# genomematt/xenomapper

Hardware: AMD Instinct MI355X
Metric: read-pairs/sec classified (higher is better)
Workload: dtype int32; 1 GPU; configs[1]: 50000000 PE 2x150 pairs/GPU, AS/XS, liberal, HBM-resident; pairs_per_gpu=50000000, step=xm_classify_compact_dev: classify+count, scan, scatter (3 launches)

## Files before the change

### xenomapper_amd/csrc/xm_kernels.hip

```cpp
#include <hip/hip_runtime.h>
#include <stdint.h>
#include <stdlib.h>

#include "xm_kernels.h"

namespace xm {

template <typename T>
__device__ __forceinline__ uint32_t mapping_state(T a1, T x1, T a2, T x2, T m)
{
    const bool low1 = a1 <= m;
    const bool low2 = a2 <= m;
    const bool prim = (a1 > m) && (low2 || a1 > a2);
    const bool sec  = (a2 > m) && (low1 || a2 > a1);
    const bool spec1 = (x1 == T(0)) || (a1 > x1);
    const bool spec2 = (x2 == T(0)) || (a2 > x2);
    uint32_t s = 6u;
    s = sec ? (spec2 ? 1u : 3u) : s;
    s = (a1 == a2) ? 4u : s;
    s = prim ? (spec1 ? 0u : 2u) : s;
    s = (low1 && low2) ? 5u : s;
    return s;
}

// ... 5 lines not shown
    const bool spec1 = (x1 == 0) || (a1 > x1);
    const bool spec2 = (x2 == 0) || (a2 > x2);
    uint32_t s = spec2 ? 1u : 3u;
    s = (gt || lt) ? s : 4u;
    s = (!low1 && (low2 || gt)) ? (spec1 ? 0u : 2u) : s;
    s = (low1 && low2) ? 5u : s;
    return s;
}

__device__ __forceinline__ uint32_t bin_of_code(int mode, uint32_t c)
{
    const uint32_t f = (c >> 3) & 7u, r = c & 7u;
    const uint32_t lo = f < r ? f : r;
    const uint32_t hi = f < r ? r : f;
    uint32_t b;
    if (mode == XM_MODE_SE) {
        b = r > 6u ? 6u : r;
    } else if (mode == XM_MODE_PE_LIBERAL) {
        b = lo;
    } else {
        b = (hi == 5u) ? 5u
          : ((hi == 4u) || (((f ^ r) & 1u) != 0u)) ? 4u
          : lo;
    }
    if (mode != XM_MODE_SE) b = (hi > 5u) ? 6u : b;
    return (c == XM_NO_UNIT) ? 7u : b;
}

template <typename T> struct Vec4;
typedef int32_t v4i32 __attribute__((ext_vector_type(4)));
typedef int32_t v4i32_a4 __attribute__((ext_vector_type(4), aligned(4)));
typedef double  v4f64 __attribute__((ext_vector_type(4)));
template <> struct Vec4<int32_t> { typedef v4i32 type; };
template <> struct Vec4<double>  { typedef v4f64 type; };

template <typename T> __device__ __forceinline__ T absent_value();
template <> __device__ __forceinline__ int32_t absent_value<int32_t>() { return INT32_MIN; }
template <> __device__ __forceinline__ double  absent_value<double>()  { return -__builtin_huge_val(); }

template <typename T, bool NT, bool FULL = false>
__device__ __forceinline__ void load4(const T *__restrict__ col, uint64_t r0, uint64_t n, T out[4])
{
    typedef typename Vec4<T>::type V;
    if (FULL || r0 + 4 <= n) {
        const V *p = reinterpret_cast<const V *>(col + r0);
        const V v = NT ? __builtin_nontemporal_load(p) : *p;
        out[0] = v.x; out[1] = v.y; out[2] = v.z; out[3] = v.w;
    } else {
#pragma unroll
        for (int j = 0; j < 4; ++j) out[j] = (r0 + j < n) ? col[r0 + j] : absent_value<T>();
    }
}

template <typename T, bool NT>
__device__ __forceinline__ void load4_wg(const T *__restrict__ wg, uint32_t byte_off, T out[4])
{
    typedef typename Vec4<T>::type V;
    const V *p = reinterpret_cast<const V *>(reinterpret_cast<const char *>(wg) + byte_off);
    const V v = NT ? __builtin_nontemporal_load(p) : *p;
    out[0] = v.x; out[1] = v.y; out[2] = v.z; out[3] = v.w;
}

__device__ __forceinline__ uint32_t wave_scan_incl(uint32_t v)
{
    v += (uint32_t)__builtin_amdgcn_update_dpp(0, (int)v, 0x111, 0xf, 0xf, false);
    v += (uint32_t)__builtin_amdgcn_update_dpp(0, (int)v, 0x112, 0xf, 0xf, false);
    v += (uint32_t)__builtin_amdgcn_update_dpp(0, (int)v, 0x114, 0xf, 0xf, false);
    v += (uint32_t)__builtin_amdgcn_update_dpp(0, (int)v, 0x118, 0xf, 0xf, false);
    v += (uint32_t)__builtin_amdgcn_update_dpp(0, (int)v, 0x142, 0xa, 0xf, false);
    v += (uint32_t)__builtin_amdgcn_update_dpp(0, (int)v, 0x143, 0xc, 0xf, false);
    return v;
}

__device__ __forceinline__ uint32_t lane_value(uint32_t v, int lane)
{
    return (uint32_t)__builtin_amdgcn_readlane((int)v, lane);
}

__device__ __forceinline__ void lds_settle()
{
    asm volatile("s_waitcnt lgkmcnt(0)" ::: "memory");
}

#define XM_HREP 8
#define XM_COUNT_LDS_WORDS (64 * XM_HREP + 16)

struct CountSink {
    uint32_t *gran_counts;
    uint32_t *part_tot;
    unsigned long long *counts_rep;
    uint8_t *bins4;
    uint32_t gran_stride;
    int mode;
    uint32_t blk0;
};

__device__ __forceinline__ void count_flush(uint32_t *lds, uint32_t granule, const CountSink &sink)
{
    const uint32_t lane = threadIdx.x & 63u;
    uint32_t *misc = lds + 64 * XM_HREP;
    const uint4 h0 = *reinterpret_cast<const uint4 *>(lds + lane * XM_HREP);
    const uint4 h1 = *reinterpret_cast<const uint4 *>(lds + lane * XM_HREP + 4);
    const uint32_t s = h0.x + h0.y + h0.z + h0.w + h1.x + h1.y + h1.z + h1.w;
    if (s != 0u) {
        atomicAdd(&sink.counts_rep[(granule % XM_COUNT_REPLICAS) * 64u + lane], (unsigned long long)s);
        atomicAdd(&misc[8u + bin_of_code(sink.mode, lane)], s);
    }
    lds_settle();
    if (lane < 8u) {
        const uint32_t v = misc[8u + lane];
        sink.gran_counts[(uint64_t)lane * sink.gran_stride + granule] = v;
        if (v != 0u) atomicAdd(&sink.part_tot[((granule & (XM_PART_REPLICAS - 1u)) * 8u + lane) * XM_PART_STRIDE + granule / XM_PART_GRAN], v);
    }
}

template <int BLOCK>
__device__ __forceinline__ void count_units(const uint32_t c[4], uint32_t *lds, const CountSink &sink)
{
    const uint32_t lane = threadIdx.x & 63u;
    const uint32_t rep = lane & (XM_HREP - 1u);
#pragma unroll
    for (int j = 0; j < 4; ++j) {
        const bool unit = c[j] != XM_NO_UNIT;
        if (__ballot(unit) == 0ull) continue;
        if (unit) atomicAdd(&lds[(c[j] & 63u) * XM_HREP + rep], 1u);
    }
    lds_settle();
    uint32_t arrived = 0;
    if (lane == 0u) arrived = atomicAdd(&lds[64 * XM_HREP], 1u);
    arrived = (uint32_t)__builtin_amdgcn_readfirstlane((int)arrived);
    if (arrived != (uint32_t)(BLOCK / 64 - 1)) return;
    lds_settle();
    count_flush(lds, blockIdx.x + sink.blk0, sink);
}

template <int MODE, bool HAS6>
__device__ __forceinline__ uint32_t unit_bin(uint32_t c)
{
    if (MODE == XM_MODE_SE) return c == XM_NO_UNIT ? 7u : (c & 7u);
    const uint32_t f = (c >> 3) & 7u, r = c & 7u;
    const uint32_t lo = f < r ? f : r, hi = f < r ? r : f;
    uint32_t b = lo;
    if (MODE == XM_MODE_PE_CONSERVATIVE) {
        b = (((f ^ r) & 1u) != 0u || hi == 4u) ? 4u : b;
        b = (hi == 5u) ? 5u : b;
    }
    if (HAS6) b = (hi > 5u) ? 6u : b;
    return c == XM_NO_UNIT ? 7u : b;
}

template <int MODE, bool HAS6>
__device__ __forceinline__ uint32_t unit_bin_of(uint32_t f, uint32_t r, bool unit)
{
    uint32_t b;
    if (MODE == XM_MODE_SE) {
        b = r;
    } else {
        const uint32_t lo = f < r ? f : r, hi = f < r ? r : f;
        b = lo;
        if (MODE == XM_MODE_PE_CONSERVATIVE) {
            b = (((f ^ r) & 1u) != 0u || hi == 4u) ? 4u : b;
            b = (hi == 5u) ? 5u : b;
        }
        if (HAS6) b = (hi > 5u) ? 6u : b;
    }
    return unit ? b : 7u;
}

template <typename T, bool PAIRED, int BLOCK, bool FULL, bool COUNTS, int BINMODE>
__device__ __forceinline__ void classify_finish(const T a1[4], const T x1[4], const T a2[4], const T x2[4], T m,
                                                uint32_t mb, uint32_t halo, uint32_t *last_state,
                                                uint8_t *__restrict__ code, uint64_t r0, uint64_t n,
                                                uint32_t *count_lds, const CountSink &sink)
{
    const uint32_t lane = threadIdx.x & 63u;
    const uint32_t wave = threadIdx.x >> 6;
    uint32_t s[4];
#pragma unroll
    for (int j = 0; j < 4; ++j) s[j] = mapping_state<T>(a1[j], x1[j], a2[j], x2[j], m);

    uint32_t c[4], fwd[4] = {0, 0, 0, 0};
    if (PAIRED) {
        uint32_t prev = (uint32_t)__builtin_amdgcn_update_dpp(0, (int)s[3], 0x138, 0xf, 0xf, false);
        if (lane == 63) last_state[wave] = s[3];
        __syncthreads();
        if (lane == 0) prev = (wave == 0) ? halo : last_state[wave - 1];
        c[0] = (mb & 1u) ? ((prev << 3) | s[0]) : XM_NO_UNIT;
        c[1] = (mb & 2u) ? ((s[0] << 3) | s[1]) : XM_NO_UNIT;
        c[2] = (mb & 4u) ? ((s[1] << 3) | s[2]) : XM_NO_UNIT;
        c[3] = (mb & 8u) ? ((s[2] << 3) | s[3]) : XM_NO_UNIT;
        fwd[0] = prev; fwd[1] = s[0]; fwd[2] = s[1]; fwd[3] = s[2];
    } else {
        if (COUNTS) __syncthreads();
#pragma unroll
        for (int j = 0; j < 4; ++j) c[j] = ((mb >> j) & 1u) ? s[j] : XM_NO_UNIT;
    }

    if (FULL || r0 + 4 <= n) {
        if (code != nullptr) *reinterpret_cast<uint32_t *>(code + r0) = c[0] | (c[1] << 8) | (c[2] << 16) | (c[3] << 24);
    } else {
#pragma unroll
        for (int j = 0; j < 4; ++j)
            if (code != nullptr && r0 + j < n) code[r0 + j] = (uint8_t)c[j];
    }
    if (BINMODE >= 0) {
        uint32_t nib = 0;
#pragma unroll
        for (int j = 0; j < 4; ++j) nib |= unit_bin_of<BINMODE, sizeof(T) == 8>(fwd[j], s[j], ((mb >> j) & 1u) != 0u) << (4 * j);
        reinterpret_cast<uint16_t *>(sink.bins4)[r0 >> 2] = (uint16_t)nib;
    }
    if (COUNTS) count_units<BLOCK>(c, count_lds, sink);
}

template <typename T, bool PAIRED, bool NT, int BLOCK, bool FULL, bool COUNTS, int BINMODE>
__device__ __forceinline__ void classify_body(const T *__restrict__ as1, const T *__restrict__ xs1,
                                              const T *__restrict__ as2, const T *__restrict__ xs2,
                                              const uint8_t *__restrict__ unit_bits8, T m,
                                              uint8_t *__restrict__ code, uint64_t n, uint32_t *last_state,
                                              uint32_t *count_lds, const CountSink &sink)
{
    const uint64_t g = (uint64_t)(blockIdx.x + sink.blk0) * BLOCK + threadIdx.x;
    const uint64_t r0 = g * 4;

    T a1[4], x1[4], a2[4], x2[4];
    load4<T, NT, FULL>(as1, r0, n, a1);
    load4<T, NT, FULL>(xs1, r0, n, x1);
    load4<T, NT, FULL>(as2, r0, n, a2);
    load4<T, NT, FULL>(xs2, r0, n, x2);
    uint32_t mb = 0;
    if (FULL || r0 < n) mb = (uint32_t)(unit_bits8[g >> 1] >> ((g & 1u) * 4u)) & 0xFu;
    if (!FULL && r0 + 4 > n) mb &= (r0 < n) ? ((1u << (uint32_t)(n - r0)) - 1u) : 0u;

    uint32_t halo = 0;
    if (PAIRED && threadIdx.x == 0) {
        if (r0 > 0) {
            const uint64_t h = r0 - 1;
            halo = mapping_state<T>(as1[h], xs1[h], as2[h], xs2[h], m);
        } else {
            mb &= ~1u;
        }
    }
    classify_finish<T, PAIRED, BLOCK, FULL, COUNTS, BINMODE>(a1, x1, a2, x2, m, mb, halo, last_state, code, r0, n, count_lds, sink);
}

template <int BLOCK>
__device__ __forceinline__ void count_lds_clear(uint32_t *count_lds)
{
    for (uint32_t k = threadIdx.x; k < (uint32_t)XM_COUNT_LDS_WORDS; k += BLOCK) count_lds[k] = 0;
}

template <typename T, bool PAIRED, bool NT, int BLOCK, bool COUNTS, int BINMODE>
__global__ void __launch_bounds__(BLOCK)
classify_kernel(const T *__restrict__ as1, const T *__restrict__ xs1,
                const T *__restrict__ as2, const T *__restrict__ xs2,
                const uint8_t *__restrict__ unit_bits8, T m,
                uint8_t *__restrict__ code, uint64_t n, CountSink sink)
{
    __shared__ uint32_t last_state[BLOCK / 64];
    __shared__ __attribute__((aligned(16))) uint32_t count_lds[COUNTS ? XM_COUNT_LDS_WORDS : 4];
    if (COUNTS) count_lds_clear<BLOCK>(count_lds);
    if (((uint64_t)blockIdx.x + sink.blk0 + 1) * (BLOCK * 4) <= n)
        classify_body<T, PAIRED, NT, BLOCK, true, COUNTS, BINMODE>(as1, xs1, as2, xs2, unit_bits8, m, code, n, last_state, count_lds, sink);
    else
        classify_body<T, PAIRED, NT, BLOCK, false, COUNTS, BINMODE>(as1, xs1, as2, xs2, unit_bits8, m, code, n, last_state, count_lds, sink);
}


__device__ __attribute__((noinline)) uint4 load_codes16_tail(const uint8_t *__restrict__ code, uint64_t base, uint64_t n)
{
    uint32_t w[4];
    for (int k = 0; k < 4; ++k) {
        uint32_t acc = 0;
        for (int j = 0; j < 4; ++j) {
            const uint64_t i = base + 4 * k + j;
            const uint32_t c = (i < n) ? (uint32_t)code[i] : XM_NO_UNIT;
            acc |= c << (8 * j);
        }
        w[k] = acc;
    }
    return make_uint4(w[0], w[1], w[2], w[3]);
}

__device__ __forceinline__ void load_codes16(const uint8_t *__restrict__ code, uint64_t base, uint64_t n,
                                             uint32_t w[4])
{
    uint4 v;
    if (base + 16 <= n) v = *reinterpret_cast<const uint4 *>(code + base);
    else v = load_codes16_tail(code, base, n);
    w[0] = v.x; w[1] = v.y; w[2] = v.z; w[3] = v.w;
}

__device__ __attribute__((noinline)) uint32_t load_codes4_tail(const uint8_t *__restrict__ code, uint64_t base, uint64_t n)
{
    uint32_t acc = 0;
    for (int j = 0; j < 4; ++j) {
        const uint64_t i = base + j;
        const uint32_t c = (i < n) ? (uint32_t)code[i] : XM_NO_UNIT;
        acc |= c << (8 * j);
    }
    return acc;
}

__global__ void __launch_bounds__(XM_BLOCK)
hist_kernel(const uint8_t *__restrict__ code, uint64_t n, uint32_t n_gran, CountSink sink)
{
    __shared__ __attribute__((aligned(16))) uint32_t lds_all[XM_BLOCK / 64][XM_COUNT_LDS_WORDS];
    const uint32_t lane = threadIdx.x & 63u, wave = threadIdx.x >> 6;
    uint32_t *lds = lds_all[wave];
    const uint32_t g = blockIdx.x * (XM_BLOCK / 64) + wave;
    if (g >= n_gran) return;
    for (uint32_t k = lane; k < (uint32_t)XM_COUNT_LDS_WORDS; k += 64u) lds[k] = 0;

    constexpr int TILES = XM_GRAN / 1024;
    const uint64_t rec0 = (uint64_t)g * XM_GRAN;
    uint32_t w[TILES][4];
#pragma unroll
    for (int k = 0; k < TILES; ++k) load_codes16(code, rec0 + (uint64_t)k * 1024u + lane * 16u, n, w[k]);
    lds_settle();

    const uint32_t rep = lane & (XM_HREP - 1u);
    uint32_t common = w[0][0] & 0xFFu;
    if (common == XM_NO_UNIT) common = (w[0][0] >> 8) & 0xFFu;
    common = (uint32_t)__builtin_amdgcn_readfirstlane((int)common);
    uint32_t n_common = 0;
#pragma unroll
    for (int k = 0; k < TILES; ++k) {
#pragma unroll
        for (int j = 0; j < 16; ++j) {
            const uint32_t c = (w[k][j >> 2] >> (8 * (j & 3))) & 0xFFu;
            const bool unit = c != XM_NO_UNIT;
            if (__ballot(unit) == 0ull) continue;
            const bool same = unit && c == common;
            n_common += same ? 1u : 0u;
            if (unit && !same) atomicAdd(&lds[(c & 63u) * XM_HREP + rep], 1u);
        }
    }
    if (n_common) atomicAdd(&lds[(common & 63u) * XM_HREP + rep], n_common);
    lds_settle();
    count_flush(lds, g, sink);
}

#define XM_SCAN_THREADS 1024
__device__ __forceinline__ unsigned long long block_sum_1024(unsigned long long v, unsigned long long *wsum)
// ... 309 lines not shown
    uint32_t base[7];
#pragma unroll
    for (int b = 0; b < 7; ++b) base[b] = lane_value(lane_base, b);
    uint32_t w[NSUB], wn[NSUB];
    load_granule(g0, w);
    if (!NIB || LISTS) lds_settle();
    for (uint32_t g = g0; g < g1; ++g) {
        if (g + 1u < g1) load_granule(g + 1u, wn);
        const uint32_t rec_g = (uint32_t)((uint64_t)g * (NSUB * 256u));
        bool staged = false;
        uint32_t cnt_g = 0;
        if (CAN_STAGE) {
            cnt_g = (lane < 7u) ? gran_counts[(uint64_t)lane * gran_stride + g] : 0u;
            uint32_t run_start, run_len;
            staged = slab_layout(cnt_g, run_start, run_len);
            if (staged) {
                uint32_t sbase[7];
#pragma unroll
                for (int b = 0; b < 7; ++b) sbase[b] = lane_value(run_start, b);
                scatter_granule<NSUB, WIDE, NIB, true, LISTS>(w, lut, rec_g, sbase, idx_out, n_units, slab, lptr);
                lds_settle();
                copy_runs_out(run_start, run_len, rec_g);
                lds_settle();
            }
        }
        if (!staged) {
            if (CAN_STAGE) {
#pragma unroll
                for (int b = 0; b < 7; ++b) base[b] = lane_value(lane_base, b);
            }
            scatter_granule<NSUB, WIDE, NIB, false, LISTS>(w, lut, rec_g, base, idx_out, n_units, slab, lptr);
        }
        if (CAN_STAGE) lane_base += cnt_g;
#pragma unroll
        for (int s = 0; s < NSUB; ++s) w[s] = wn[s];
    }
}

#define XM_RUNS_WCNT_AT (64 * XM_HREP)
#define XM_RUNS_SLAB_AT (XM_RUNS_WCNT_AT + 64)
#define XM_RUNS_LDS_WORDS (XM_RUNS_SLAB_AT + XM_GRAN / 2)

struct RunsSink {
    uint16_t *runs16;
    uint16_t *gran_counts16;
    unsigned long long *counts_rep;
};

template <int SLOTS, int NB>
__device__ __forceinline__ uint32_t runs_ranks(const uint32_t bin[4], uint32_t pos[4])
{
    const uint32_t lane = threadIdx.x & 63u;
    uint32_t wc = 0;
#pragma unroll
    for (int b = 0; b < NB; ++b) {
        uint64_t m[4], any = 0;
#pragma unroll
        for (int j = 0; j < 4; ++j) {
            m[j] = ((SLOTS >> j) & 1) ? __ballot(bin[j] == (uint32_t)b) : 0ull;
            any |= m[j];
        }
        if (any == 0ull) continue;
        uint32_t t = 0, total = 0;
#pragma unroll
        for (int j = 0; j < 4; ++j)
            if ((SLOTS >> j) & 1) { t = mbcnt64(m[j], t); total += (uint32_t)__builtin_popcountll(m[j]); }
#pragma unroll
        for (int j = 0; j < 4; ++j)
            if ((SLOTS >> j) & 1) pos[j] = (bin[j] == (uint32_t)b) ? t : pos[j];
        wc = (lane == (uint32_t)b) ? total : wc;
    }
#pragma unroll
    for (int j = 1; j < 4; ++j)
#pragma unroll
        for (int i = 0; i < j; ++i)
            if (((SLOTS >> j) & 1) && ((SLOTS >> i) & 1)) pos[j] += (bin[i] == bin[j]) ? 1u : 0u;
    return wc;
}

template <typename T, bool PAIRED, bool NT, int BLOCK, bool FULL, int BINMODE>
__device__ __forceinline__ void classify_runs_body(const T *__restrict__ as1, const T *__restrict__ xs1,
                                                   const T *__restrict__ as2, const T *__restrict__ xs2,
                                                   const uint8_t *__restrict__ unit_bits8, T m, uint64_t n,
                                                   uint32_t *last_state, uint32_t *lds, const RunsSink &rs)
{
    static_assert(BLOCK == 512 && BLOCK * 4 == XM_GRAN, "eight waves, one granule");
    constexpr bool HAS6 = sizeof(T) == 8;
    constexpr int NB = HAS6 ? 7 : 6;
    const uint32_t lane = threadIdx.x & 63u;
    const uint32_t wave = (uint32_t)__builtin_amdgcn_readfirstlane((int)(threadIdx.x >> 6));
    const uint32_t g = blockIdx.x;
    const uint64_t g4 = (uint64_t)blockIdx.x * BLOCK + threadIdx.x;
    const uint64_t r0 = g4 * 4;
    T a1[4], x1[4], a2[4], x2[4];
    load4<T, NT, FULL>(as1, r0, n, a1);
    load4<T, NT, FULL>(xs1, r0, n, x1);
    load4<T, NT, FULL>(as2, r0, n, a2);
    load4<T, NT, FULL>(xs2, r0, n, x2);
    uint32_t mb = 0;
    if (FULL || r0 < n) mb = (uint32_t)(unit_bits8[g4 >> 1] >> ((g4 & 1u) * 4u)) & 0xFu;
    if (!FULL && r0 + 4 > n) mb &= (r0 < n) ? ((1u << (uint32_t)(n - r0)) - 1u) : 0u;
    uint32_t halo = 0;
    if (PAIRED && threadIdx.x == 0) {
        if (r0 > 0) {
            const uint64_t h = r0 - 1;
            halo = mapping_state<T>(as1[h], xs1[h], as2[h], xs2[h], m);
        } else {
            mb &= ~1u;
        }
    }
    uint32_t s[4];
#pragma unroll
    for (int j = 0; j < 4; ++j) s[j] = mapping_state<T>(a1[j], x1[j], a2[j], x2[j], m);
    uint32_t c[4], fwd[4] = {0, 0, 0, 0};
    if (PAIRED) {
        uint32_t prev = (uint32_t)__builtin_amdgcn_update_dpp(0, (int)s[3], 0x138, 0xf, 0xf, false);
        if (lane == 63) last_state[wave] = s[3];
        __syncthreads();
        if (lane == 0) prev = (wave == 0) ? halo : last_state[wave - 1];
        c[0] = (mb & 1u) ? ((prev << 3) | s[0]) : XM_NO_UNIT;
        c[1] = (mb & 2u) ? ((s[0] << 3) | s[1]) : XM_NO_UNIT;
        c[2] = (mb & 4u) ? ((s[1] << 3) | s[2]) : XM_NO_UNIT;
        c[3] = (mb & 8u) ? ((s[2] << 3) | s[3]) : XM_NO_UNIT;
        fwd[0] = prev; fwd[1] = s[0]; fwd[2] = s[1]; fwd[3] = s[2];
    } else {
        __syncthreads();
#pragma unroll
        for (int j = 0; j < 4; ++j) c[j] = ((mb >> j) & 1u) ? s[j] : XM_NO_UNIT;
    }
    uint32_t bin[4];
#pragma unroll
    for (int j = 0; j < 4; ++j) bin[j] = unit_bin_of<BINMODE, HAS6>(fwd[j], s[j], ((mb >> j) & 1u) != 0u);
    {
        const uint32_t rep = lane & (XM_HREP - 1u);
#pragma unroll
        for (int j = 0; j < 4; ++j) {
            const bool unit = c[j] != XM_NO_UNIT;
            if (__ballot(unit) == 0ull) continue;
            if (unit) atomicAdd(&lds[(c[j] & 63u) * XM_HREP + rep], 1u);
        }
    }
    uint32_t pos[4] = {0, 0, 0, 0};
    const bool inter = PAIRED && __ballot((mb & 5u) != 0u) == 0ull;
    const uint32_t wc = inter ? runs_ranks<0xA, NB>(bin, pos) : runs_ranks<0xF, NB>(bin, pos);
    uint32_t *wave_cnt = lds + XM_RUNS_WCNT_AT;
    uint16_t *slab = reinterpret_cast<uint16_t *>(lds + XM_RUNS_SLAB_AT);
    if (lane < 8u) wave_cnt[wave * 8u + lane] = wc;
    __syncthreads();
    uint32_t off, tot;
    {
        const uint32_t v = wave_cnt[lane];
        off = (lane >> 3) < wave ? v : 0u;
        tot = v;
        off += (uint32_t)__shfl_xor((int)off, 8, 64);  tot += (uint32_t)__shfl_xor((int)tot, 8, 64);
        off += (uint32_t)__shfl_xor((int)off, 16, 64); tot += (uint32_t)__shfl_xor((int)tot, 16, 64);
        off += (uint32_t)__shfl_xor((int)off, 32, 64); tot += (uint32_t)__shfl_xor((int)tot, 32, 64);
    }
    const uint32_t t8 = lane < 8u ? tot : 0u;
    const uint32_t incl8 = wave_scan_incl(t8);
    const uint32_t where = incl8 - t8 + off;
    const uint32_t units = lane_value(incl8, 7);
#pragma unroll
    for (int j = 0; j < 4; ++j) {
        uint32_t at = 0;
#pragma unroll
        for (int b = 0; b < NB; ++b) at = (bin[j] == (uint32_t)b) ? lane_value(where, b) : at;
        if (bin[j] < 7u) slab[at + pos[j]] = (uint16_t)(threadIdx.x * 4u + (uint32_t)j);
    }
    __syncthreads();
    if (threadIdx.x < (uint32_t)(XM_GRAN / 8) && threadIdx.x * 8u < units)
        reinterpret_cast<uint4 *>(rs.runs16 + (uint64_t)g * XM_GRAN)[threadIdx.x] = reinterpret_cast<const uint4 *>(slab)[threadIdx.x];
    if (wave == 0u) {
        if (lane < 8u) rs.gran_counts16[(uint64_t)g * 8u + lane] = (uint16_t)tot;
        const uint4 h0 = *reinterpret_cast<const uint4 *>(lds + lane * XM_HREP);
        const uint4 h1 = *reinterpret_cast<const uint4 *>(lds + lane * XM_HREP + 4);
        const uint32_t sum = h0.x + h0.y + h0.z + h0.w + h1.x + h1.y + h1.z + h1.w;
        if (sum != 0u) atomicAdd(&rs.counts_rep[(g % XM_COUNT_REPLICAS) * 64u + lane], (unsigned long long)sum);
    }
}

template <typename T, bool PAIRED, bool NT, int BLOCK, int BINMODE>
__global__ void __launch_bounds__(BLOCK)
classify_runs_kernel(const T *__restrict__ as1, const T *__restrict__ xs1, const T *__restrict__ as2, const T *__restrict__ xs2,
                     const uint8_t *__restrict__ unit_bits8, T m, uint64_t n, RunsSink rs)
{
    __shared__ uint32_t last_state[BLOCK / 64];
    __shared__ __attribute__((aligned(16))) uint32_t lds[XM_RUNS_LDS_WORDS];
    for (uint32_t q = threadIdx.x; q < 64u * XM_HREP; q += BLOCK) lds[q] = 0;
    if (((uint64_t)blockIdx.x + 1) * (BLOCK * 4) <= n)
        classify_runs_body<T, PAIRED, NT, BLOCK, true, BINMODE>(as1, xs1, as2, xs2, unit_bits8, m, n, last_state, lds, rs);
    else
        classify_runs_body<T, PAIRED, NT, BLOCK, false, BINMODE>(as1, xs1, as2, xs2, unit_bits8, m, n, last_state, lds, rs);
}

__global__ void __launch_bounds__(256)
runs_finish_kernel(unsigned long long *__restrict__ counts_rep, unsigned long long *__restrict__ counts,
                   unsigned long long *__restrict__ n_out, int mode)
{
    __shared__ unsigned long long part[4][64];
    __shared__ unsigned long long bins[8];
    const uint32_t slot = threadIdx.x & 63u, q = threadIdx.x >> 6;
    unsigned long long acc = 0;
#pragma unroll
    for (uint32_t r = 0; r < XM_COUNT_REPLICAS / 4u; ++r) {
        acc += counts_rep[(q * (XM_COUNT_REPLICAS / 4u) + r) * 64u + slot];
        counts_rep[(q * (XM_COUNT_REPLICAS / 4u) + r) * 64u + slot] = 0;
    }
    part[q][slot] = acc;
    if (threadIdx.x < 8u) bins[threadIdx.x] = 0;
    __syncthreads();
    if (q == 0u) {
        const unsigned long long v = part[0][slot] + part[1][slot] + part[2][slot] + part[3][slot];
        counts[slot] = v;
        if (v != 0ull) {
            atomicAdd(&bins[bin_of_code(mode, slot)], v);
            atomicAdd(&bins[7], v);
        }
    }
    __syncthreads();
    if (threadIdx.x < 8u) n_out[threadIdx.x] = bins[threadIdx.x];
}

__global__ void __launch_bounds__(XM_BLOCK)
cigar_kernel(uint64_t n, const int32_t *__restrict__ nm, const uint32_t *__restrict__ cig_off,
             const uint32_t *__restrict__ cig_oplen, int32_t *__restrict__ as_out,
             uint32_t *__restrict__ range_flag)
{
    const uint64_t stride = (uint64_t)gridDim.x * XM_BLOCK;
    for (uint64_t i = (uint64_t)blockIdx.x * XM_BLOCK + threadIdx.x; i < n; i += stride) {
        const int32_t nmv = nm[i];
        int32_t out = INT32_MIN;
        if (nmv != INT32_MIN) {
            long long s = -6ll * (long long)nmv;
            const uint32_t k1 = cig_off[i + 1];
            for (uint32_t k = cig_off[i]; k < k1; ++k) {
                const uint32_t v = cig_oplen[k];
                const uint32_t op = v & 15u;
                const long long len = (long long)(v >> 4);
                s -= (op == 1u || op == 2u) ? (5ll + 3ll * len) : 0ll;
                s -= (op == 4u) ? 2ll * len : 0ll;
            }
            if (s <= (long long)INT32_MIN || s > (long long)INT32_MAX) {
                if (range_flag) atomicOr(range_flag, 1u);
                s = s < 0 ? (long long)INT32_MIN + 1 : (long long)INT32_MAX;
            }
            out = (int32_t)s;
        }
        as_out[i] = out;
    }
}

#define XM_CIG_SPEC 3

__device__ __forceinline__ long long cigar_term(uint32_t v)
{
    const uint32_t op = v & 15u;
    const long long len = (long long)(v >> 4);
    long long t = (op == 1u || op == 2u) ? (5ll + 3ll * len) : 0ll;
    t += (op == 4u) ? 2ll * len : 0ll;
    return t;
}

__device__ __forceinline__ uint32_t cigar_term32(uint32_t v)
{
    const uint32_t op = v & 15u, len = v >> 4;
    uint32_t t = (op == 1u || op == 2u) ? (5u + 3u * len) : 0u;
    t += (op == 4u) ? 2u * len : 0u;
    return t;
}

__device__ __forceinline__ uint32_t cigar_term24(uint32_t v)
{
    uint32_t op = v & 15u;
    op = op < 8u ? op : 8u;
    const uint32_t a = __builtin_amdgcn_ubfe(0x00000550u, op * 4u, 4u);
// ... 513 lines not shown
                acc = acc + prod;
            }
        } else {
            for (uint32_t j = 0; j < mm; ++j) {
                const double prod = tile[t + j] * density[j0 + j];
                const double s = acc + prod;
                acc = (j < lim) ? s : acc;
            }
        }
    }
    if (i < n) out[i] = (track[i] == 1.0) ? 1.0 : acc;
}

__global__ void __launch_bounds__(XM_CLASSIFY_BLOCK)
stream_probe_kernel(const v4i32 *__restrict__ c0, const v4i32 *__restrict__ c1, const v4i32 *__restrict__ c2,
                    const v4i32 *__restrict__ c3, uint16_t *__restrict__ out, uint64_t n_groups)
{
    const uint64_t g = (uint64_t)blockIdx.x * XM_CLASSIFY_BLOCK + threadIdx.x;
    if (g >= n_groups) return;
    const v4i32 a = __builtin_nontemporal_load(c0 + g), b = __builtin_nontemporal_load(c1 + g);
    const v4i32 c = __builtin_nontemporal_load(c2 + g), d = __builtin_nontemporal_load(c3 + g);
    const v4i32 x = a ^ b ^ c ^ d;
    out[g] = (uint16_t)(x.x ^ x.y ^ x.z ^ x.w);
}

void launch_stream_probe(hipStream_t st, uint64_t n, const int32_t *c0, const int32_t *c1, const int32_t *c2, const int32_t *c3,
                         uint8_t *out)
{
    const uint64_t n_groups = n / 4;
    const uint32_t grid = (uint32_t)((n_groups + XM_CLASSIFY_BLOCK - 1) / XM_CLASSIFY_BLOCK);
    if (grid == 0) return;
    stream_probe_kernel<<<grid, XM_CLASSIFY_BLOCK, 0, st>>>(reinterpret_cast<const v4i32 *>(c0), reinterpret_cast<const v4i32 *>(c1),
                                                            reinterpret_cast<const v4i32 *>(c2), reinterpret_cast<const v4i32 *>(c3),
                                                            reinterpret_cast<uint16_t *>(out), n_groups);
}

static_assert(XM_CLASSIFY_BLOCK * 4 == XM_GRAN, "the counting classify workgroup is one granule");

GranPlan plan_granules(uint64_t n)
{
    GranPlan p;
    uint64_t g = (n + XM_GRAN - 1) / XM_GRAN;
    if (g == 0) g = 1;
    p.n_gran = (uint32_t)g;
    p.gran_stride = (p.n_gran + 63u) & ~63u;
    return p;
}

static CountSink make_sink(const CountPlan *cp, int mode)
{
    CountSink s;
    s.gran_counts = cp ? cp->gran_counts : nullptr;
    s.part_tot = cp ? cp->part_tot : nullptr;
    s.counts_rep = cp ? reinterpret_cast<unsigned long long *>(cp->counts_rep) : nullptr;
    s.bins4 = cp ? cp->bins4 : nullptr;
    s.gran_stride = cp ? cp->plan.gran_stride : 0u;
    s.mode = mode;
    s.blk0 = cp ? cp->gran0 : 0u;
    return s;
}

template <typename T>
static void launch_classify_t(hipStream_t st, int mode, uint64_t n,
                              const T *as1, const T *xs1, const T *as2, const T *xs2,
                              const uint64_t *unit_bits, T m, uint8_t *code, const CountPlan *cp)
{
    const uint64_t per_block = (uint64_t)XM_CLASSIFY_BLOCK * 4;
    static_assert(XM_CLASSIFY_BLOCK * 4 == XM_GRAN, "a counting workgroup is a granule: CountPlan's chunk is in both");
    const uint32_t all = (uint32_t)((n + per_block - 1) / per_block);
    const uint32_t grid = (cp && cp->gran1) ? cp->gran1 - cp->gran0 : all;
    const uint8_t *bits8 = reinterpret_cast<const uint8_t *>(unit_bits);
    const CountSink sink = make_sink(cp, mode);
    const bool paired = mode != XM_MODE_SE;
#define XM_LAUNCH_CLS(P, C, B) classify_kernel<T, P, XM_CLASSIFY_NT, XM_CLASSIFY_BLOCK, C, B><<<grid, XM_CLASSIFY_BLOCK, 0, st>>>(as1, xs1, as2, xs2, bits8, m, code, n, sink)
    if (cp && cp->bins4) {
        if (mode == XM_MODE_SE) XM_LAUNCH_CLS(false, true, XM_MODE_SE);
        else if (mode == XM_MODE_PE_LIBERAL) XM_LAUNCH_CLS(true, true, XM_MODE_PE_LIBERAL);
        else XM_LAUNCH_CLS(true, true, XM_MODE_PE_CONSERVATIVE);
    }
    else if (cp) { if (paired) XM_LAUNCH_CLS(true, true, -1); else XM_LAUNCH_CLS(false, true, -1); }
    else         { if (paired) XM_LAUNCH_CLS(true, false, -1); else XM_LAUNCH_CLS(false, false, -1); }
#undef XM_LAUNCH_CLS
}

void launch_classify_i32(hipStream_t st, int mode, uint64_t n,
                         const int32_t *as1, const int32_t *xs1, const int32_t *as2, const int32_t *xs2,
                         const uint64_t *unit_bits, int32_t m, uint8_t *code, const CountPlan *cp)
{
    launch_classify_t<int32_t>(st, mode, n, as1, xs1, as2, xs2, unit_bits, m, code, cp);
}

void launch_classify_f64(hipStream_t st, int mode, uint64_t n,
                         const double *as1, const double *xs1, const double *as2, const double *xs2,
                         const uint64_t *unit_bits, double m, uint8_t *code, const CountPlan *cp)
{
    launch_classify_t<double>(st, mode, n, as1, xs1, as2, xs2, unit_bits, m, code, cp);
}

template <typename T>
static void launch_classify_runs_t(hipStream_t st, int mode, uint64_t n,
                                   const T *as1, const T *xs1, const T *as2, const T *xs2,
                                   const uint64_t *unit_bits, T m, const RunsOut &ro)
{
    const uint64_t per_block = (uint64_t)XM_CLASSIFY_BLOCK * 4;
    const uint32_t grid = (uint32_t)((n + per_block - 1) / per_block);
    const uint8_t *bits8 = reinterpret_cast<const uint8_t *>(unit_bits);
    RunsSink rs;
    rs.runs16 = ro.runs16;
    rs.gran_counts16 = ro.gran_counts16;
    rs.counts_rep = reinterpret_cast<unsigned long long *>(ro.counts_rep);
#define XM_LAUNCH_RUNS(P, B) classify_runs_kernel<T, P, XM_CLASSIFY_NT, XM_CLASSIFY_BLOCK, B><<<grid, XM_CLASSIFY_BLOCK, 0, st>>>(as1, xs1, as2, xs2, bits8, m, n, rs)
    if (mode == XM_MODE_SE) XM_LAUNCH_RUNS(false, XM_MODE_SE);
    else if (mode == XM_MODE_PE_LIBERAL) XM_LAUNCH_RUNS(true, XM_MODE_PE_LIBERAL);
    else XM_LAUNCH_RUNS(true, XM_MODE_PE_CONSERVATIVE);
#undef XM_LAUNCH_RUNS
}

void launch_classify_runs_i32(hipStream_t st, int mode, uint64_t n,
                              const int32_t *as1, const int32_t *xs1, const int32_t *as2, const int32_t *xs2,
                              const uint64_t *unit_bits, int32_t m, const RunsOut &ro)
{
    launch_classify_runs_t<int32_t>(st, mode, n, as1, xs1, as2, xs2, unit_bits, m, ro);
}

void launch_classify_runs_f64(hipStream_t st, int mode, uint64_t n,
                              const double *as1, const double *xs1, const double *as2, const double *xs2,
                              const uint64_t *unit_bits, double m, const RunsOut &ro)
{
    launch_classify_runs_t<double>(st, mode, n, as1, xs1, as2, xs2, unit_bits, m, ro);
}

void launch_runs_finish(hipStream_t st, int mode, uint64_t *counts_rep, uint64_t *counts, uint64_t *n_out)
{
    runs_finish_kernel<<<1, 256, 0, st>>>(reinterpret_cast<unsigned long long *>(counts_rep),
                                          reinterpret_cast<unsigned long long *>(counts),
                                          reinterpret_cast<unsigned long long *>(n_out), mode);
}

void launch_classify_cigar(hipStream_t st, int mode, uint64_t n,
                           const int32_t *nm1, const uint32_t *off1, const uint32_t *ops1, const int32_t *xs1,
                           const int32_t *nm2, const uint32_t *off2, const uint32_t *ops2, const int32_t *xs2,
                           const uint64_t *unit_bits, int32_t m, uint8_t *code, uint32_t *range_flag)
{
    const uint64_t per_block = (uint64_t)XM_CIGAR_BLOCK * 4;
    const uint32_t grid = (uint32_t)((n + per_block - 1) / per_block);
    const uint8_t *bits8 = reinterpret_cast<const uint8_t *>(unit_bits);
    if (mode == XM_MODE_SE)
        classify_cigar_kernel<false, XM_CIGAR_BLOCK><<<grid, XM_CIGAR_BLOCK, 0, st>>>(
            nm1, off1, ops1, xs1, nm2, off2, ops2, xs2, bits8, m, code, n, range_flag);
    else
        classify_cigar_kernel<true, XM_CIGAR_BLOCK><<<grid, XM_CIGAR_BLOCK, 0, st>>>(
            nm1, off1, ops1, xs1, nm2, off2, ops2, xs2, bits8, m, code, n, range_flag);
}

void launch_classify_cigp(hipStream_t st, int mode, uint64_t n, const CigCols &s1, const CigCols &s2,
                          const uint64_t *unit_bits, int32_t m, uint8_t *code, uint32_t *range_flag, const CountPlan &cp)
{
    const uint64_t per_block = (uint64_t)XM_CIGP_BLOCK * 4;
    const uint32_t grid = (uint32_t)((n + per_block - 1) / per_block);
    const uint32_t n_tiles = (uint32_t)((n + 255) / 256);
    const uint8_t *bits8 = reinterpret_cast<const uint8_t *>(unit_bits);
    const CountSink sink = make_sink(&cp, mode);
#define XM_LAUNCH_CIGP(P, B) classify_cigp_kernel<P, XM_CIGP_BLOCK, true, B><<<grid, XM_CIGP_BLOCK, 0, st>>>(s1, s2, bits8, m, code, n, n_tiles, range_flag, sink)
    if (cp.bins4) {
        if (mode == XM_MODE_SE) XM_LAUNCH_CIGP(false, XM_MODE_SE);
        else if (mode == XM_MODE_PE_LIBERAL) XM_LAUNCH_CIGP(true, XM_MODE_PE_LIBERAL);
// ... 77 lines not shown
```

Before: 144.4 billion read-pairs/s.

## Compute per-wave halo state directly and drop cross-wave LDS handoff barrier

Each wave now loads the record just before its first row itself (lanes 0-3 fetch the four columns, then broadcast via readlane) and computes the boundary mapping state locally. This removes the LDS last_state exchange and the __syncthreads before classification, and drops the serialized thread-0 halo load. The LDS histogram clear moves after the loads are issued, with a raw s_barrier so global loads stay in flight across the barrier. Optional timeline instrumentation and a variant switch are added behind macros. Each wave adds a few redundant global loads in exchange.

```diff
diff --git a/xenomapper_amd/csrc/xm_kernels.hip b/xenomapper_amd/csrc/xm_kernels.hip
--- a/xenomapper_amd/csrc/xm_kernels.hip
+++ b/xenomapper_amd/csrc/xm_kernels.hip
@@ -111,6 +111,35 @@
     asm volatile("s_waitcnt lgkmcnt(0)" ::: "memory");
 }
 
+__device__ __forceinline__ void barrier_loads_in_flight()
+{
+    asm volatile("s_barrier" ::: "memory");
+    __builtin_amdgcn_sched_barrier(0);
+}
+
+#ifndef XM_K1_VARIANT
+#define XM_K1_VARIANT 1
+#endif
+#ifdef XM_K1_TIMELINE
+__device__ unsigned long long *xm_k1_tl_buf;
+__device__ unsigned long long xm_k1_tl_cap;
+#define XM_TL_DECL unsigned long long xm_tl[5] = {0, 0, 0, 0, 0}
+#define XM_TL(k) do { __builtin_amdgcn_sched_barrier(0); xm_tl[k] = wall_clock64(); __builtin_amdgcn_sched_barrier(0); } while (0)
+#define XM_TL_DATA() do { asm volatile("s_waitcnt vmcnt(0)" ::: "memory"); XM_TL(2); } while (0)
+#define XM_TL_FLUSH(wg, waves)                                                                                   \
+    do {                                                                                                         \
+        if ((threadIdx.x & 63u) == 0u && xm_k1_tl_buf != nullptr && (unsigned long long)(wg) < xm_k1_tl_cap) {   \
+            unsigned long long *tl_p = xm_k1_tl_buf + ((unsigned long long)(wg) * (waves) + (threadIdx.x >> 6)) * 5u; \
+            for (int tl_k = 0; tl_k < 5; ++tl_k) tl_p[tl_k] = xm_tl[tl_k];                                       \
+        }                                                                                                        \
+    } while (0)
+#else
+#define XM_TL_DECL
+#define XM_TL(k) ((void)0)
+#define XM_TL_DATA() ((void)0)
+#define XM_TL_FLUSH(wg, waves) ((void)0)
+#endif
+
 #define XM_HREP 8
 #define XM_COUNT_LDS_WORDS (64 * XM_HREP + 16)
 
@@ -196,14 +225,17 @@
     return unit ? b : 7u;
 }
 
-template <typename T, bool PAIRED, int BLOCK, bool FULL, bool COUNTS, int BINMODE>
+enum { XM_FRONT_LDS = 0, XM_FRONT_WAVE = 1 };
+
+template <typename T, bool PAIRED, int BLOCK, bool FULL, bool COUNTS, int BINMODE, int FRONT = XM_FRONT_LDS>
 __device__ __forceinline__ void classify_finish(const T a1[4], const T x1[4], const T a2[4], const T x2[4], T m,
                                                 uint32_t mb, uint32_t halo, uint32_t *last_state,
                                                 uint8_t *__restrict__ code, uint64_t r0, uint64_t n,
-                                                uint32_t *count_lds, const CountSink &sink)
+                                                uint32_t *count_lds, const CountSink &sink, unsigned long long *xm_tl = nullptr)
 {
     const uint32_t lane = threadIdx.x & 63u;
     const uint32_t wave = threadIdx.x >> 6;
+    if (xm_tl) XM_TL_DATA();
     uint32_t s[4];
 #pragma unroll
     for (int j = 0; j < 4; ++j) s[j] = mapping_state<T>(a1[j], x1[j], a2[j], x2[j], m);
@@ -211,16 +243,21 @@
     uint32_t c[4], fwd[4] = {0, 0, 0, 0};
     if (PAIRED) {
         uint32_t prev = (uint32_t)__builtin_amdgcn_update_dpp(0, (int)s[3], 0x138, 0xf, 0xf, false);
-        if (lane == 63) last_state[wave] = s[3];
-        __syncthreads();
-        if (lane == 0) prev = (wave == 0) ? halo : last_state[wave - 1];
+        if (FRONT == XM_FRONT_WAVE) {
+            prev = (lane == 0) ? halo : prev;
+        } else {
+            if (lane == 63) last_state[wave] = s[3];
+            __syncthreads();
+            if (xm_tl) XM_TL(3);
+            if (lane == 0) prev = (wave == 0) ? halo : last_state[wave - 1];
+        }
         c[0] = (mb & 1u) ? ((prev << 3) | s[0]) : XM_NO_UNIT;
         c[1] = (mb & 2u) ? ((s[0] << 3) | s[1]) : XM_NO_UNIT;
         c[2] = (mb & 4u) ? ((s[1] << 3) | s[2]) : XM_NO_UNIT;
         c[3] = (mb & 8u) ? ((s[2] << 3) | s[3]) : XM_NO_UNIT;
         fwd[0] = prev; fwd[1] = s[0]; fwd[2] = s[1]; fwd[3] = s[2];
     } else {
-        if (COUNTS) __syncthreads();
+        if (COUNTS && FRONT == XM_FRONT_LDS) __syncthreads();
 #pragma unroll
         for (int j = 0; j < 4; ++j) c[j] = ((mb >> j) & 1u) ? s[j] : XM_NO_UNIT;
     }
@@ -239,6 +276,49 @@
         reinterpret_cast<uint16_t *>(sink.bins4)[r0 >> 2] = (uint16_t)nib;
     }
     if (COUNTS) count_units<BLOCK>(c, count_lds, sink);
+}
+
+
+template <typename T, bool FULL>
+__device__ __forceinline__ T front_record_load(const T *__restrict__ as1, const T *__restrict__ xs1,
+                                               const T *__restrict__ as2, const T *__restrict__ xs2,
+                                               uint64_t t0, uint64_t n)
+{
+    const uint32_t lane = threadIdx.x & 63u;
+    uint64_t h = t0 - (t0 != 0 ? 1u : 0u);
+    if (!FULL) h = h < n ? h : n - 1;
+    T v = T(0);
+    if (lane < 4u) {
+        const T *col = lane == 0u ? as1 : lane == 1u ? xs1 : lane == 2u ? as2 : xs2;
+        v = col[h];
+    }
+    return v;
+}
+
+__device__ __forceinline__ int32_t lane_bcast(int32_t v, int k) { return __builtin_amdgcn_readlane(v, k); }
+__device__ __forceinline__ double lane_bcast(double v, int k)
+{
+    return __hiloint2double(__builtin_amdgcn_readlane(__double2hiint(v), k), __builtin_amdgcn_readlane(__double2loint(v), k));
+}
+
+template <typename T>
+__device__ __forceinline__ uint32_t front_record_state(T v, T m)
+{
+    return mapping_state<T>(lane_bcast(v, 0), lane_bcast(v, 1), lane_bcast(v, 2), lane_bcast(v, 3), m);
+}
+
+template <int BLOCK>
+__device__ __forceinline__ void count_lds_clear(uint32_t *count_lds)
+{
+    for (uint32_t k = threadIdx.x; k < (uint32_t)XM_COUNT_LDS_WORDS; k += BLOCK) count_lds[k] = 0;
+}
+
+template <int BLOCK>
+__device__ __forceinline__ void count_lds_clear_flat(uint32_t *count_lds)
+{
+    static_assert(XM_COUNT_LDS_WORDS > BLOCK && XM_COUNT_LDS_WORDS <= 2 * BLOCK, "one word per thread, a second for some");
+    count_lds[threadIdx.x] = 0;
+    if (threadIdx.x < (uint32_t)(XM_COUNT_LDS_WORDS - BLOCK)) count_lds[BLOCK + threadIdx.x] = 0;
 }
 
 template <typename T, bool PAIRED, bool NT, int BLOCK, bool FULL, bool COUNTS, int BINMODE>
@@ -248,34 +328,57 @@
                                               uint8_t *__restrict__ code, uint64_t n, uint32_t *last_state,
                                               uint32_t *count_lds, const CountSink &sink)
 {
+    XM_TL_DECL;
+    XM_TL(0);
+    const uint32_t wave = (uint32_t)__builtin_amdgcn_readfirstlane((int)(threadIdx.x >> 6));
     const uint64_t g = (uint64_t)(blockIdx.x + sink.blk0) * BLOCK + threadIdx.x;
     const uint64_t r0 = g * 4;
+    const uint64_t t0 = ((uint64_t)(blockIdx.x + sink.blk0) * BLOCK + wave * 64u) * 4;
 
     T a1[4], x1[4], a2[4], x2[4];
     load4<T, NT, FULL>(as1, r0, n, a1);
     load4<T, NT, FULL>(xs1, r0, n, x1);
     load4<T, NT, FULL>(as2, r0, n, a2);
     load4<T, NT, FULL>(xs2, r0, n, x2);
-    uint32_t mb = 0;
-    if (FULL || r0 < n) mb = (uint32_t)(unit_bits8[g >> 1] >> ((g & 1u) * 4u)) & 0xFu;
+    uint32_t mask_byte = 0;
+    if (FULL || r0 < n) mask_byte = unit_bits8[g >> 1];
+    T fv = T(0);
+#if XM_K1_VARIANT == 2
+    if (PAIRED && wave == 0u) fv = front_record_load<T, FULL>(as1, xs1, as2, xs2, t0, n);
+    if (COUNTS) count_lds_clear_flat<BLOCK>(count_lds);
+    XM_TL(1);
+    __builtin_amdgcn_sched_barrier(0);
+#else
+    if (PAIRED) fv = front_record_load<T, FULL>(as1, xs1, as2, xs2, t0, n);
+    if (COUNTS) {
+        count_lds_clear_flat<BLOCK>(count_lds);
+        lds_settle();
+    }
+    XM_TL(1);
+    if (COUNTS) barrier_loads_in_flight();
+    else __builtin_amdgcn_sched_barrier(0);
+    XM_TL(3);
+    XM_TL_DATA();
+#endif
+
+    uint32_t mb = (mask_byte >> ((g & 1u) * 4u)) & 0xFu;
     if (!FULL && r0 + 4 > n) mb &= (r0 < n) ? ((1u << (uint32_t)(n - r0)) - 1u) : 0u;
-
-    uint32_t halo = 0;
-    if (PAIRED && threadIdx.x == 0) {
-        if (r0 > 0) {
-            const uint64_t h = r0 - 1;
-            halo = mapping_state<T>(as1[h], xs1[h], as2[h], xs2[h], m);
-        } else {
-            mb &= ~1u;
-        }
-    }
-    classify_finish<T, PAIRED, BLOCK, FULL, COUNTS, BINMODE>(a1, x1, a2, x2, m, mb, halo, last_state, code, r0, n, count_lds, sink);
-}
-
-template <int BLOCK>
-__device__ __forceinline__ void count_lds_clear(uint32_t *count_lds)
-{
-    for (uint32_t k = threadIdx.x; k < (uint32_t)XM_COUNT_LDS_WORDS; k += BLOCK) count_lds[k] = 0;
+    uint32_t front = 0;
+    if (PAIRED) {
+        if (r0 == 0) mb &= ~1u;
+        front = front_record_state<T>(fv, m);
+    }
+#if XM_K1_VARIANT == 2
+#ifdef XM_K1_TIMELINE
+    classify_finish<T, PAIRED, BLOCK, FULL, COUNTS, BINMODE, XM_FRONT_LDS>(a1, x1, a2, x2, m, mb, front, last_state, code, r0, n, count_lds, sink, xm_tl);
+#else
+    classify_finish<T, PAIRED, BLOCK, FULL, COUNTS, BINMODE, XM_FRONT_LDS>(a1, x1, a2, x2, m, mb, front, last_state, code, r0, n, count_lds, sink);
+#endif
+#else
+    classify_finish<T, PAIRED, BLOCK, FULL, COUNTS, BINMODE, XM_FRONT_WAVE>(a1, x1, a2, x2, m, mb, front, nullptr, code, r0, n, count_lds, sink);
+#endif
+    XM_TL(4);
+    XM_TL_FLUSH(blockIdx.x + sink.blk0, BLOCK / 64);
 }
 
 template <typename T, bool PAIRED, bool NT, int BLOCK, bool COUNTS, int BINMODE>
@@ -287,7 +390,6 @@
 {
     __shared__ uint32_t last_state[BLOCK / 64];
     __shared__ __attribute__((aligned(16))) uint32_t count_lds[COUNTS ? XM_COUNT_LDS_WORDS : 4];
-    if (COUNTS) count_lds_clear<BLOCK>(count_lds);
     if (((uint64_t)blockIdx.x + sink.blk0 + 1) * (BLOCK * 4) <= n)
         classify_body<T, PAIRED, NT, BLOCK, true, COUNTS, BINMODE>(as1, xs1, as2, xs2, unit_bits8, m, code, n, last_state, count_lds, sink);
     else
@@ -763,7 +865,7 @@
 __device__ __forceinline__ void classify_runs_body(const T *__restrict__ as1, const T *__restrict__ xs1,
                                                    const T *__restrict__ as2, const T *__restrict__ xs2,
                                                    const uint8_t *__restrict__ unit_bits8, T m, uint64_t n,
-                                                   uint32_t *last_state, uint32_t *lds, const RunsSink &rs)
+                                                   uint32_t *lds, const RunsSink &rs)
 {
     static_assert(BLOCK == 512 && BLOCK * 4 == XM_GRAN, "eight waves, one granule");
     constexpr bool HAS6 = sizeof(T) == 8;
@@ -778,34 +880,31 @@
     load4<T, NT, FULL>(xs1, r0, n, x1);
     load4<T, NT, FULL>(as2, r0, n, a2);
     load4<T, NT, FULL>(xs2, r0, n, x2);
-    uint32_t mb = 0;
-    if (FULL || r0 < n) mb = (uint32_t)(unit_bits8[g4 >> 1] >> ((g4 & 1u) * 4u)) & 0xFu;
+    uint32_t mask_byte = 0;
+    if (FULL || r0 < n) mask_byte = unit_bits8[g4 >> 1];
+    T fv = T(0);
+    if (PAIRED) fv = front_record_load<T, FULL>(as1, xs1, as2, xs2, ((uint64_t)blockIdx.x * BLOCK + wave * 64u) * 4, n);
+    static_assert(64 * XM_HREP == BLOCK, "one histogram word per thread");
+    lds[threadIdx.x] = 0;
+    lds_settle();
+    barrier_loads_in_flight();
+    uint32_t mb = (mask_byte >> ((g4 & 1u) * 4u)) & 0xFu;
     if (!FULL && r0 + 4 > n) mb &= (r0 < n) ? ((1u << (uint32_t)(n - r0)) - 1u) : 0u;
-    uint32_t halo = 0;
-    if (PAIRED && threadIdx.x == 0) {
-        if (r0 > 0) {
-            const uint64_t h = r0 - 1;
-            halo = mapping_state<T>(as1[h], xs1[h], as2[h], xs2[h], m);
-        } else {
-            mb &= ~1u;
-        }
-    }
+    if (PAIRED && r0 == 0) mb &= ~1u;
     uint32_t s[4];
 #pragma unroll
     for (int j = 0; j < 4; ++j) s[j] = mapping_state<T>(a1[j], x1[j], a2[j], x2[j], m);
     uint32_t c[4], fwd[4] = {0, 0, 0, 0};
     if (PAIRED) {
         uint32_t prev = (uint32_t)__builtin_amdgcn_update_dpp(0, (int)s[3], 0x138, 0xf, 0xf, false);
-        if (lane == 63) last_state[wave] = s[3];
-        __syncthreads();
-        if (lane == 0) prev = (wave == 0) ? halo : last_state[wave - 1];
+        const uint32_t front = front_record_state<T>(fv, m);
+        prev = (lane == 0) ? front : prev;
         c[0] = (mb & 1u) ? ((prev << 3) | s[0]) : XM_NO_UNIT;
         c[1] = (mb & 2u) ? ((s[0] << 3) | s[1]) : XM_NO_UNIT;
         c[2] = (mb & 4u) ? ((s[1] << 3) | s[2]) : XM_NO_UNIT;
         c[3] = (mb & 8u) ? ((s[2] << 3) | s[3]) : XM_NO_UNIT;
         fwd[0] = prev; fwd[1] = s[0]; fwd[2] = s[1]; fwd[3] = s[2];
     } else {
-        __syncthreads();
 #pragma unroll
         for (int j = 0; j < 4; ++j) c[j] = ((mb >> j) & 1u) ? s[j] : XM_NO_UNIT;
     }
@@ -865,13 +964,11 @@
 classify_runs_kernel(const T *__restrict__ as1, const T *__restrict__ xs1, const T *__restrict__ as2, const T *__restrict__ xs2,
                      const uint8_t *__restrict__ unit_bits8, T m, uint64_t n, RunsSink rs)
 {
-    __shared__ uint32_t last_state[BLOCK / 64];
     __shared__ __attribute__((aligned(16))) uint32_t lds[XM_RUNS_LDS_WORDS];
-    for (uint32_t q = threadIdx.x; q < 64u * XM_HREP; q += BLOCK) lds[q] = 0;
     if (((uint64_t)blockIdx.x + 1) * (BLOCK * 4) <= n)
-        classify_runs_body<T, PAIRED, NT, BLOCK, true, BINMODE>(as1, xs1, as2, xs2, unit_bits8, m, n, last_state, lds, rs);
+        classify_runs_body<T, PAIRED, NT, BLOCK, true, BINMODE>(as1, xs1, as2, xs2, unit_bits8, m, n, lds, rs);
     else
-        classify_runs_body<T, PAIRED, NT, BLOCK, false, BINMODE>(as1, xs1, as2, xs2, unit_bits8, m, n, last_state, lds, rs);
+        classify_runs_body<T, PAIRED, NT, BLOCK, false, BINMODE>(as1, xs1, as2, xs2, unit_bits8, m, n, lds, rs);
 }
 
 __global__ void __launch_bounds__(256)
@@ -1551,6 +1648,15 @@
     else         { if (paired) XM_LAUNCH_CLS(true, false, -1); else XM_LAUNCH_CLS(false, false, -1); }
 #undef XM_LAUNCH_CLS
 }
+
+#ifdef XM_K1_TIMELINE
+extern "C" int xm_k1_timeline_set(void *buf, unsigned long long n_workgroups)
+{
+    unsigned long long *p = static_cast<unsigned long long *>(buf);
+    if (hipMemcpyToSymbol(HIP_SYMBOL(xm_k1_tl_cap), &n_workgroups, sizeof n_workgroups) != hipSuccess) return -1;
+    return hipMemcpyToSymbol(HIP_SYMBOL(xm_k1_tl_buf), &p, sizeof p) == hipSuccess ? 0 : -1;
+}
+#endif
 
 void launch_classify_i32(hipStream_t st, int mode, uint64_t n,
                          const int32_t *as1, const int32_t *xs1, const int32_t *as2, const int32_t *xs2,
```

Measured after the change: 134.8 billion read-pairs/s. -6.7%, worse.
